# mycophonic/saprobe-alac

Hardware: AMD Instinct MI355X
Metric: Msamples/s decoded (16-bit stereo, 4096-frame packets) (higher is better)
Workload: dtype int32; 1 GPU; 65536 packets/GPU x 16-bit 2-ch 4096-frame ALAC, music-like synthetic, device-resident in/out; packets_per_gpu=65536

## Files before the change

saprobe-alac_amd/csrc/alac_duo.h:

```cpp
#ifndef ALAC_DUO_H
#define ALAC_DUO_H

#include <type_traits>

#include "alac_regular.h"

namespace alac {

#ifndef ALAC_WRAP_COUNTDOWN
#define ALAC_WRAP_COUNTDOWN 0
#endif
#ifndef ALAC_DUO_CHUNK
#define ALAC_DUO_CHUNK 16
#endif
constexpr uint32_t DUO_CHUNK = ALAC_DUO_CHUNK;
static_assert(DUO_CHUNK % 16u == 0u && DUO_CHUNK <= 32u, "a writer's half chunk is whole groups of 8 steps and fits a stager row");
constexpr int DUO_UN8_MAX = 12;
enum { ROLE_A = 0, ROLE_B = 1, ROLE_BOTH = 2, ROLE_C = 3 };

template <class W, class B, int NA, int OUT, int ROLE, bool F16, bool NARROW, bool EA, bool UN8W = false, bool EC = false, int WMODE = 0>
ALAC_DEV void duo_phase(W& wv, const DevCfg& cfg, const B& bits, RegLane<W>& s, uint32_t size, uint32_t ns,
                        uint32_t n_it, uint32_t hdr_pos, uint32_t den_shift, uint32_t chan_bits, int32_t mix_res,
                        uint32_t mix_sh, uint32_t na_rt, uint32_t shift_pos, uint32_t sb, uint32_t mode) {
    constexpr bool DO_A = ROLE == ROLE_A || ROLE == ROLE_BOTH, DO_B = ROLE == ROLE_B || ROLE == ROLE_BOTH;
    constexpr bool RAW = OUT == OUT_RAW;
    constexpr bool LAST = OUT == OUT_STEREO || OUT == OUT_MONO || RAW;
    constexpr bool CPE = OUT == OUT_STEREO;
    constexpr bool QND = W::kResMem || EC;
    constexpr bool GEN = NA == 0;
    constexpr int NR = GEN ? 1 : NA;
    constexpr bool WRAP = !(NA == 4 || NA == 5 || NA == 6 || NA == 8);
    constexpr uint32_t BIAS = 0x80000000u;
    static_assert(!(EA && EC), "one writer");
    constexpr bool DO_C = (ROLE == ROLE_C || ROLE == ROLE_BOTH) && EC;
    constexpr bool EMIT_A = (EA || EC) && LAST && !RAW;
    constexpr bool DO_EMIT = EMIT_A ? (EC ? DO_C : DO_A) : DO_B;
    constexpr uint32_t CH = EMIT_A ? DUO_CHUNK / 2u : DUO_CHUNK;
    constexpr bool U16_OUT = F16 && EC && OUT == OUT_UTILE;
    constexpr bool C16 = F16 && EC && CPE && EMIT_A;
    const uint32_t na = GEN ? na_rt : (uint32_t)NA;
#ifdef ALAC_SYNC_DIAG
    wv.dg_phase = LAST ? 1u : 0u;
#endif
    uint32_t kb = cfg.kb;
    ALAC_OWN_REG(kb);
    const uint32_t wb = go_shl(1u, kb) - 1u;
    const uint32_t c31kb = 31u - kb;
    const uint32_t chan_shift = 32u - chan_bits;
    const int32_t den_half = den_shift ? (int32_t)(1u << (den_shift - 1u)) : 0;
    const uint32_t rnd_neg = (1u << den_shift) - 1u;

    int32_t coef[NR];
    uint32_t hb[NR + 1];
    if (DO_B) {
#pragma unroll
        for (int j = 0; j < NR; ++j)
            coef[j] = (!GEN || ((uint32_t)j < na && na != 31)) ? (int32_t)(int16_t)bits.get(hdr_pos + 16u + 16u * (uint32_t)j, 16) : 0;
#pragma unroll
        for (int j = 0; j <= NR; ++j) hb[j] = BIAS;
    }
    uint64_t pk_acc = 0;
    uint32_t pk_n = 0;
    const uint32_t bps = cfg.bps;
    const uint64_t pk_msk = bps == 4 ? 0xffffffffull : ((1ull << (8u * bps)) - 1ull);
    const bool merge_any = DO_EMIT && LAST && !F16 && !RAW && wv.any(sb != 0);
    const bool mode_any = DO_B && wv.any(mode != 0);
    int32_t dprev = 0;
    auto prepass = [&](uint32_t idx, int32_t del) -> int32_t {
        if (!mode_any) return del;
        const int32_t dd = idx == 0 ? del : sext_cs(del + dprev, chan_shift);
        dprev = mode != 0 ? dd : dprev;
        return mode != 0 ? dd : del;
    };
    constexpr bool MID_ONLY = !NARROW && WMODE == 1;
    const bool mid = !NARROW && (MID_ONLY || !wv.any(ns != 0u && chan_bits > 25u));
    auto predict = [&](int32_t del, auto wrap) -> int32_t {
        constexpr bool WR = decltype(wrap)::value;
        if (NARROW) return predict_narrow<NR, GEN, WR, !RAW>(coef, hb, na, del, den_shift, den_half, rnd_neg, chan_shift);
        if (MID_ONLY || mid) return predict_narrow<NR, GEN, WR, !RAW, true>(coef, hb, na, del, den_shift, den_half, rnd_neg, chan_shift);
        if constexpr (!MID_ONLY) return predict_wide<NR, GEN, WR>(coef, hb, na, del, den_shift, den_half, chan_shift);
        return 0;
    };
    auto predict_q = [&](int32_t x, auto wrap) -> int32_t {
        constexpr bool WR = decltype(wrap)::value;
        if (!QND) return predict(x, wrap);
        if (NARROW) return predict_narrow_nd<NR, GEN, WR, !RAW>(coef, hb, na, (uint32_t)x, den_shift, den_half, rnd_neg, chan_shift);
        return predict(gol_unfold((uint32_t)x), wrap);
    };
    using wrap_yes = std::integral_constant<bool, WRAP>;
    using wrap_no = std::integral_constant<bool, false>;
    const uint32_t nzm = mix_res != 0 ? 0xffffffffu : 0u;

    uint32_t ns_live = s.err == 0 ? ns : 0u;
    if (DO_A) gol_head(s, c31kb);
    auto qval = [&](uint32_t nd) -> int32_t { return QND ? (int32_t)nd : gol_unfold(nd); };
    auto golomb_chunk = [&](uint32_t c) {
        const uint32_t buf = c & 1u;
        if ((c + 1u) * CH <= n_it) {
#pragma nounroll
            for (uint32_t g = 0; g < CH; g += GOL_TICK) {
                s.rd.tick(wv, s.pos);
                s.near = gol_near(s, c * CH + g, ns_live);
#pragma nounroll
                for (uint32_t h = g; h < g + GOL_TICK; h += 4u) {
#pragma unroll
                    for (uint32_t j = 0; j < 4u; ++j)
                        wv.rq_write(buf, h + j, qval(gol_step<true>(wv, bits, s, size, kb, wb, c31kb, chan_bits, c * CH + h + j, ns, ns_live)));
                }
            }
            return;
        }
#pragma nounroll
        for (uint32_t j = 0; j < CH; ++j) {
            const uint32_t i = c * CH + j;
            if (i >= n_it) break;
            if ((i & (GOL_TICK - 1u)) == 0) {
                s.rd.tick(wv, s.pos);
                s.near = gol_near(s, i, ns_live);
            }
            wv.rq_write(buf, j, qval(gol_step<true>(wv, bits, s, size, kb, wb, c31kb, chan_bits, i, ns, ns_live)));
        }
    };
    constexpr bool FP_OK = F16 && CPE && LAST && !EMIT_A && !RAW;
    uint32_t fp_base = 0, fp_inc = 0;
    using fp_yes = std::integral_constant<bool, true>;
    using fp_no = std::integral_constant<bool, false>;
    auto emit = [&](uint32_t i, int32_t o, int32_t u, uint64_t sw, uint32_t jj, auto fp) {
        constexpr bool FP = decltype(fp)::value;
        const bool on = i < ns;
        if (RAW) {
            wv.st_push_if((uint32_t)o, on);
            return;
        }
        int32_t l = o, r = 0;
        if (CPE) {
            const int32_t vv = o;
            const int32_t mv = NARROW ? ALAC_MUL24(mix_res, vv) : (int32_t)((uint32_t)mix_res * (uint32_t)vv);
            l = u + (int32_t)((uint32_t)vv & nzm) - (mv >> mix_sh);
            r = (int32_t)((((uint32_t)(l - vv)) & nzm) | ((uint32_t)vv & ~nzm));
        }
        if (F16) {
            const uint32_t pcm = ((uint32_t)l & 0xffffu) | ((uint32_t)r << 16);
            if (FP) wv.st_put(fp_base, jj, pcm, fp_inc);
            else wv.st_push_if(pcm, on);
            return;
        }
        if (cfg.bit_depth == 20) {
            l = (int32_t)((uint32_t)l << 4);
            r = (int32_t)((uint32_t)r << 4);
        }
        if (merge_any) {
            const uint32_t sh_l = sb ? (uint32_t)(sw >> (64u - sb)) : 0u;
            const uint32_t sh_r = (CPE && sb) ? (uint32_t)((sw << sb) >> (64u - sb)) : 0u;
            l = (int32_t)((uint32_t)l << sb) | (int32_t)sh_l;
            r = (int32_t)((uint32_t)r << sb) | (int32_t)sh_r;
        }
        {
            pk_acc |= ((uint64_t)(uint32_t)l & pk_msk) << (8u * pk_n);
            pk_n += on ? bps : 0u;
            bool em = pk_n >= 4u;
            wv.st_push_if((uint32_t)pk_acc, em);
            pk_acc = em ? pk_acc >> 32 : pk_acc;
            pk_n = em ? pk_n - 4u : pk_n;
            if (CPE) {
                pk_acc |= ((uint64_t)(uint32_t)r & pk_msk) << (8u * pk_n);
                pk_n += on ? bps : 0u;
                em = pk_n >= 4u;
                wv.st_push_if((uint32_t)pk_acc, em);
                pk_acc = em ? pk_acc >> 32 : pk_acc;
                pk_n = em ? pk_n - 4u : pk_n;
            }
            pk_acc &= pk_n ? ((1ull << (8u * pk_n)) - 1ull) : 0ull;
        }
    };
    uint32_t u_even = 0;
    auto put = [&](uint32_t buf, uint32_t j, uint32_t i, int32_t o, int32_t u, uint64_t sw, uint32_t jj, auto fp) {
#pragma unroll
        for (int t = NR; t >= 1; --t) hb[t] = hb[t - 1];
        hb[0] = (uint32_t)o ^ BIAS;
        if (!LAST && U16_OUT) {
            if (i & 1u) *wv.u_row(i >> 1) = (int32_t)ALAC_PACK_LO16(u_even, o);
            else if (i + 1u == n_it) *wv.u_row(i >> 1) = o;
            else u_even = (uint32_t)o;
        } else if (!LAST) *wv.u_row(i) = o;
        else if (EMIT_A) wv.rq_write(buf, CH + j, o);
        else emit(i, o, u, sw, jj, fp);
    };
    constexpr bool PK3 = CPE && LAST && !F16 && !RAW && !EMIT_A;
    constexpr bool PK3C = CPE && LAST && !F16 && !RAW && EMIT_A && EC;
    const bool sb8 = (PK3 || PK3C) && !wv.any(ns != 0u && sb != 8u);
    const bool sb0 = (PK3 || PK3C) && !wv.any(ns != 0u && sb != 0u);
    const bool pk3 = (PK3 || PK3C) && bps == 3u && (sb8 || sb0);
    const uint32_t sh_byte = shift_pos >> 3, sh_bit = shift_pos & 7u;
    auto pk3_block = [&](uint32_t rowq, const int32_t (&vv4)[4], const int32_t (&uu4)[4], uint32_t g0, uint32_t g1, uint32_t g2) {
        const uint32_t w0 = (uint32_t)(((((uint64_t)g0) << 32) | g1) << sh_bit >> 32);
        const uint32_t w1 = (uint32_t)(((((uint64_t)g1) << 32) | g2) << sh_bit >> 32);
        uint32_t lq[4], rq[4];
#pragma unroll
        for (uint32_t j = 0; j < 4u; ++j) {
            const int32_t vv = vv4[j];
            const int32_t mv = NARROW ? ALAC_MUL24(mix_res, vv) : (int32_t)((uint32_t)mix_res * (uint32_t)vv);
            int32_t l = uu4[j] + (int32_t)((uint32_t)vv & nzm) - (mv >> mix_sh);
            int32_t r = (int32_t)((((uint32_t)(l - vv)) & nzm) | ((uint32_t)vv & ~nzm));
            if (sb8) {
                const uint32_t w = j < 2u ? w0 : w1;
// ... 235 lines not shown
                        for (uint32_t j = 0; j < UN; ++j) {
                            const int32_t o = predict_q(dv[j], wrap);
#pragma unroll
                            for (int t = NR; t >= 1; --t) hb[t] = hb[t - 1];
                            hb[0] = (uint32_t)o ^ BIAS;
                            if (j & 1u) ub[(ptrdiff_t)(j >> 1) * rs] = (int32_t)ALAC_PACK_LO16(u_even, o);
                            else u_even = (uint32_t)o;
                        }
                        continue;
                    }
#pragma unroll
                    for (uint32_t j = 0; j < UN; ++j)
                        put(buf, g + j, c * CH + g + j, predict_q(dv[j], wrap), uv[j], sv[j], j, fp);
                    if (FP) wv.st_advance(fp_inc);
                    if (LAST && !EMIT_A) wv.st_step();
                }
            };
            auto run_groups = [&](auto wrap) {
                if (FP_OK) {
                    const uint32_t c_end = (c + 1u) * CH;
                    const bool ends_here = ns > c * CH && ns < c_end;
                    if (!wv.any(ends_here)) {
                        fp_inc = ns >= c_end ? UN : 0u;
                        groups(wrap, fp_yes{});
                        return;
                    }
                    groups(wrap, fp_no{});
                    if (ends_here) (void)wv.st_finish();
                    return;
                }
                groups(wrap, fp_no{});
            };
#if !ALAC_WRAP_COUNTDOWN
            if (WRAP) {
                constexpr uint32_t T = 32767u - CH;
                uint32_t far = 0;
#pragma unroll
                for (int j = 0; j < NR; ++j) far = umax(far, (uint32_t)coef[j] + T);
                if (!wv.any(far > 2u * T)) {
                    run_groups(wrap_no{});
                    return;
                }
            }
#else
            if (WRAP) {
                if (wrap_safe == 0u) {
                    uint32_t mag = 0;
#pragma unroll
                    for (int j = 0; j < NR; ++j) mag = umax(mag, (uint32_t)(coef[j] ^ (coef[j] >> 31)));
                    wrap_safe = (32767u - wv.max_u32(mag)) / CH;
                }
                if (wrap_safe != 0u) {
                    --wrap_safe;
                    run_groups(wrap_no{});
                    return;
                }
            }
#endif
            run_groups(wrap_yes{});
            return;
        }
#if ALAC_WRAP_COUNTDOWN
        wrap_safe = 0;
#endif
#pragma nounroll
        for (uint32_t j = 0; j < CH; ++j) {
            const uint32_t i = c * CH + j;
            if (i >= n_it) break;
            const int32_t qv = wv.rq_read(buf, j);
            const int32_t del = prepass(i, QND ? gol_unfold((uint32_t)qv) : qv);
            int32_t o;
            if (i == 0 || (GEN && na == 0)) o = del;
            else if (i <= na || (GEN && na == 31)) o = sext_cs(del + (int32_t)(hb[0] ^ BIAS), chan_shift);
            else o = predict(del, wrap_yes{});
            put(buf, j, i, o, (CPE && !EMIT_A) ? *wv.u_row(i) : 0,
                (!EMIT_A && merge_any) ? bits.window_raw(shift_pos + i * sstep) : 0ull, 0u, fp_no{});
            if (LAST && !EMIT_A) wv.st_step();
            if (FP_OK && i + 1u == ns) (void)wv.st_finish();
        }
    };

    const uint32_t nch = (n_it + CH - 1u) / CH;
    const uint32_t iters = nch + (EMIT_A ? 2u : 1u);
    for (uint32_t c = 0; c < iters; ++c) {
        if (DO_A) {
            if (EMIT_A && !EC && c >= 2u) fetch_chunk(c - 2u);
            if (c < nch) golomb_chunk(c);
        }
        if (DO_B) {
            if (c >= 1u && c <= nch) predict_chunk(c - 1u);
        }
        if (DO_A && EMIT_A && !EC) {
            if (c >= 2u) emit_chunk(c - 2u);
        }
        if (DO_C && C16) {
            if (c >= 2u) emit_chunk16(c - 2u);
            if (c >= 1u && c <= nch) fetch_u16(c - 1u);
        } else if (DO_C && EMIT_A) {
            if (c >= 2u) {
#pragma unroll
                for (uint32_t j = 0; j < CH; ++j) {
                    u_v[j] = u_n[j];
                    sw_v[j] = sw_n[j];
                }
#pragma unroll
                for (uint32_t q = 0; q < CH / 4u; ++q) {
                    g_v[q][0] = g_n[q][0];
                    g_v[q][1] = g_n[q][1];
                    g_v[q][2] = g_n[q][2];
                }
            }
            if (c >= 1u && c <= nch) fetch_mem_ahead(c - 1u);
            if (c >= 2u) {
                fetch_chunk(c - 2u);
                emit_chunk(c - 2u);
            }
        }
        wv.duo_sync();
    }
    if (DO_EMIT && LAST) wv.st_tail(pk_acc, pk_n);
    if (!LAST) wv.duo_sync_mem();
}

template <class W, class B, int T, int OUT, int LPP, int NAC = 0, bool U16 = false>
ALAC_DEV void duo_phase_lanes(W& wv, const B& bits, uint32_t q, uint32_t n_it, uint32_t hdr_pos, uint32_t den_shift,
                              uint32_t chan_bits, uint32_t na_rt) {
    static_assert(LPP == 2 || LPP == 4, "lanes per packet");
    static_assert(LPP == 2 ? NAC == 0 : (NAC >= 1 && (NAC + 3) / 4 == T), "four lanes: T = ceil(order / 4)");
    const uint32_t na = NAC != 0 ? (uint32_t)NAC : na_rt;
    constexpr bool LAST = OUT != OUT_UTILE;
    constexpr uint32_t CH = LAST ? DUO_CHUNK / 2u : DUO_CHUNK;
    constexpr uint32_t BIAS = 0x80000000u;
    const bool wraps = order_wraps16(na);
    const uint32_t chan_shift = 32u - chan_bits;
    const int32_t den_half = den_shift ? (int32_t)(1u << (den_shift - 1u)) : 0;
    const int32_t dh0 = q == 0u ? den_half : 0;
    const uint32_t rnd_neg = (1u << den_shift) - 1u;
    const uint32_t q0m = q == 0u ? 0xffffffffu : 0u;
    const uint32_t up1 = q < 3u ? 0xffffffffu : 0u, up2 = q < 2u ? 0xffffffffu : 0u, up3 = q < 1u ? 0xffffffffu : 0u;
    int32_t coef[T], wneg[T], m[T];
    uint32_t g[T + 1];
#pragma unroll
    for (int t = 0; t < T; ++t) {
        const uint32_t jt = q * (uint32_t)T + (uint32_t)t;
        const bool have = jt < na;
        coef[t] = have ? (int32_t)(int16_t)bits.get(hdr_pos + 16u + 16u * jt, 16) : 0;
        wneg[t] = have ? -(int32_t)(na - jt) : 0;
        m[t] = have ? 1 : 0;
        g[t] = BIAS;
    }
    g[T] = BIAS;
    int32_t prev = 0;
    constexpr int QTOP = NAC != 0 ? (NAC - 1) / T : 1, TTOP = NAC != 0 ? NAC - QTOP * T : T;
    const bool top_last = na == 2u * (uint32_t)T;

    auto step = [&](uint32_t i, uint32_t nd, auto plain_c, auto wrap_c) -> int32_t {
        constexpr bool PLAIN = decltype(plain_c)::value, WR = decltype(wrap_c)::value;
        uint32_t topb;
        if constexpr (LPP == 2) topb = wv.pair_hi(top_last ? g[T] : g[T - 1]);
        else topb = wv.template quad_from<QTOP>(g[TTOP]);
        const uint32_t nsg = nd & 1u, sgnm = 0u - nsg, hm = nd >> 1;
        const int32_t del = (int32_t)(hm ^ sgnm);
        int32_t rem = (int32_t)(hm + nsg);
        if (!PLAIN) {
            if (i <= na) rem = 0;
        }
        const uint32_t rnd = rnd_neg & sgnm;
        int32_t acc = dh0, s = 0;
        int32_t e[T], sg[T];
        uint32_t qv[T];
#pragma unroll
        for (int t = T - 1; t >= 0; --t) {
            e[t] = (int32_t)(g[t] - topb);
            const uint32_t ae = ALAC_SAD(topb, g[t], rnd);
            sg[t] = ALAC_SIGN(e[t]);
            qv[t] = ae >> den_shift;
            if (t != 0) {
                acc = ALAC_MAD24(coef[t], e[t], acc);
                s = ALAC_MAD24(qv[t], wneg[t], s);
            } else {
                acc = ALAC_MUL24(coef[t], e[t]) + acc;
                s = ALAC_MUL24((int32_t)qv[t], wneg[t]) + s;
            }
        }
        if (LPP == 2) rem += (int32_t)(wv.pair_hi((uint32_t)s) & q0m);
        else rem += (int32_t)((wv.template quad_up<1>((uint32_t)s) & up1) + (wv.template quad_up<2>((uint32_t)s) & up2) +
                              (wv.template quad_up<3>((uint32_t)s) & up3));
#pragma unroll
        for (int t = T - 1; t >= 0; --t) {
            const int32_t go = ALAC_MED3_0(rem, m[t]);
            const int32_t delta = (int32_t)ALAC_XAD(sg[t], sgnm, nsg);
            rem = ALAC_MAD24(qv[t], wneg[t], rem);
            int32_t cj = ALAC_MAD24(delta, go, coef[t]);
            if (WR) cj = (int32_t)(int16_t)cj;
            coef[t] = cj;
        }
        const int32_t at = LPP == 2 ? wv.pair_sum(acc) : wv.quad_sum(acc);
        int32_t o = ALAC_SEXT_BITS(del + (int32_t)(topb ^ BIAS) + (at >> den_shift), chan_bits);
        if (!PLAIN) {
            if (i == 0u) o = del;
            else if (i <= na) o = sext_cs(del + prev, chan_shift);
        }
// ... 280 lines not shown
```

saprobe-alac_amd/csrc/alac_regular.h:

```cpp
#ifndef ALAC_REGULAR_H
#define ALAC_REGULAR_H

#include "alac_wave.h"

#ifndef ALAC_NOINLINE
#define ALAC_NOINLINE
#endif
#ifndef ALAC_UNLIKELY
#define ALAC_UNLIKELY(x) __builtin_expect(!!(x), 0)
#endif
#ifndef ALAC_HD
#define ALAC_HD ALAC_DEV
#endif
#ifndef ALAC_SAD
#define ALAC_SAD(a, b, c) (((a) > (b) ? (a) - (b) : (b) - (a)) + (c))
#endif
#ifndef ALAC_LOAD4
#define ALAC_LOAD4(q, a, b, c, d) \
    do {                         \
        (a) = (q)[0];            \
        (b) = (q)[1];            \
        (c) = (q)[2];            \
        (d) = (q)[3];            \
    } while (0)
// ... 48 lines not shown
#endif
#ifndef ALAC_NOT_ADD
#define ALAC_NOT_ADD(a, c) (~(uint32_t)(a) + (uint32_t)(c))
#endif
#ifndef ALAC_ALIGNBIT
#define ALAC_ALIGNBIT(hi, lo, sh) ((uint32_t)(((((uint64_t)(uint32_t)(hi)) << 32) | (uint32_t)(lo)) >> ((sh) & 31u)))
#endif
#ifndef ALAC_MULHI
#define ALAC_MULHI(a, b) ((uint32_t)(((uint64_t)(uint32_t)(a) * (uint64_t)(uint32_t)(b)) >> 32))
#endif
#ifndef ALAC_BFE
#define ALAC_BFE(x, off, width) ((((uint32_t)(x)) >> ((off) & 31u)) & ((1u << ((width) & 31u)) - 1u))
#endif
#ifndef ALAC_PACK_LO16
#define ALAC_PACK_LO16(x, y) ((((uint32_t)(x)) & 0xffffu) | (((uint32_t)(y)) << 16))
#endif
#ifndef ALAC_PACK_HI16
#define ALAC_PACK_HI16(x, y) ((((uint32_t)(x)) >> 16) | (((uint32_t)(y)) & 0xffff0000u))
#endif
#ifndef ALAC_PK_ADD16
#define ALAC_PK_ADD16(a, b) \
    (((((uint32_t)(a)) + ((uint32_t)(b))) & 0xffffu) | (((((uint32_t)(a)) >> 16) + (((uint32_t)(b)) >> 16)) << 16))
#endif
#ifndef ALAC_PK_SUB16
#define ALAC_PK_SUB16(a, b) \
    (((((uint32_t)(a)) - ((uint32_t)(b))) & 0xffffu) | (((((uint32_t)(a)) >> 16) - (((uint32_t)(b)) >> 16)) << 16))
#endif

namespace alac {

constexpr uint32_t KEY_WIDE = 1024;
constexpr uint32_t KEY_IRREGULAR = 2048;
constexpr uint32_t NUM_KEYS = 2049;

ALAC_DEV bool regular_order(uint32_t na) { return na <= 16 || na == 31; }
ALAC_DEV int32_t imax(int32_t a, int32_t b) { return a > b ? a : b; }

ALAC_HD bool lean_config(const DevCfg& cfg) { return cfg.kb != 0 && cfg.pb <= 73u; }

ALAC_DEV uint32_t classify_regular(const DevCfg& cfg, const uint8_t* pkt, uint32_t size, uint32_t avail) {
    if (cfg.num_channels > 2 || cfg.aligned16 == 0 || !lean_config(cfg) ||
        cfg.frame_length > 65536u || cfg.frame_length <= 32u)
        return KEY_IRREGULAR;
    const Bits bits{pkt, size, avail};
    if (size < 12) return KEY_IRREGULAR;
    const uint32_t tag = bits.get(0, 3);
    const bool cpe = cfg.num_channels == 2;
    if (cpe ? tag != 1 : !(tag == 0 || tag == 3)) return KEY_IRREGULAR;
    if (bits.get(7, 12) != 0) return KEY_IRREGULAR;
    const uint32_t hdr = bits.get(19, 4);
    if (hdr & 1u) return KEY_IRREGULAR;
    const uint32_t bs = (hdr >> 1) & 3u;
    if (bs == 3) return KEY_IRREGULAR;
    const uint32_t chan_bits = cfg.bit_depth - 8u * bs + (cpe ? 1u : 0u);
    if (chan_bits < 1 || chan_bits > 33 || cfg.bit_depth < 8u * bs) return KEY_IRREGULAR;
    const uint32_t wide = chan_bits > 23u ? KEY_WIDE : 0u;
    uint32_t pos = 23;
    uint32_t ns = cfg.frame_length;
    if (hdr >> 3) {
        ns = bits.get(pos, 32);
        pos += 32;
    }
    if (ns == 0 || ns > cfg.frame_length) return KEY_IRREGULAR;
    pos += 16;
    const uint32_t hu = bits.get(pos, 16);
    const uint32_t nu = hu & 0x1fu;
    if ((hu >> 12) != 0 || !regular_order(nu)) return KEY_IRREGULAR;
    pos += 16u + 16u * nu;
    uint32_t nv = 0;
    if (cpe) {
        const uint32_t hv = bits.get(pos, 16);
        nv = hv & 0x1fu;
        if ((hv >> 12) != 0 || !regular_order(nv)) return KEY_IRREGULAR;
        pos += 16u + 16u * nv;
    }
    const uint64_t ent = (uint64_t)pos + (uint64_t)bs * 8u * (cpe ? 2u : 1u) * ns;
    if ((ent >> 3) >= size || (bs != 0 && (ent >> 3) + 10u > size)) return KEY_IRREGULAR;
    return nu * 32u + nv + wide;
}

#ifndef ALAC_RING_START_AHEAD
#define ALAC_RING_START_AHEAD 0
#endif
template <class W>
struct RingRd {
    const uint32_t* base;
    uint32_t bias;
    uint32_t end_b;
    uint32_t full;
    uint32_t wa, wb;
    uint32_t fill;
    static constexpr uint32_t RING = W::kRingDw;
    static_assert(RING >= 32, "blocks of 8 dwords need a ring of 32");
    uint32_t p0, p1, p2, p3, p4, p5, p6, p7;
    bool pend;

    ALAC_DEV void init(const uint8_t* pkt, uint32_t size) {
        const uint32_t mis = (uint32_t)(reinterpret_cast<uintptr_t>(pkt) & 3u);
        base = reinterpret_cast<const uint32_t*>(pkt - mis);
        bias = mis * 8u;
        end_b = size ? mis + size : 0u;
        full = end_b >> 2;
        wa = wb = fill = 0;
        p0 = p1 = p2 = p3 = p4 = p5 = p6 = p7 = 0;
        pend = false;
    }
    ALAC_DEV uint32_t tail1(uint32_t idx) const {
        const uint32_t last = end_b ? (end_b - 1u) >> 2 : 0u;
        const uint32_t v = base[umin(idx, last)];
        const uint32_t lo = idx * 4u;
        const uint32_t nb = end_b > lo ? umin(end_b - lo, 4u) : 0u;
        return v & (nb >= 4u ? 0xffffffffu : ((1u << (8u * nb)) - 1u));
    }
    ALAC_DEV void load8(uint32_t at) {
        if (at + 8u <= full) {
            ALAC_LOAD4(base + at, p0, p1, p2, p3);
            ALAC_LOAD4(base + at + 4u, p4, p5, p6, p7);
        } else {
            p0 = tail1(at);
            p1 = tail1(at + 1u);
            p2 = tail1(at + 2u);
            p3 = tail1(at + 3u);
            p4 = tail1(at + 4u);
            p5 = tail1(at + 5u);
            p6 = tail1(at + 6u);
            p7 = tail1(at + 7u);
        }
    }
    ALAC_DEV void commit(W& wv) {
        const uint32_t slot = fill & (RING - 1u);
        const uint32_t d0 = __builtin_bswap32(p0);
        wv.ring_write4(slot, d0, __builtin_bswap32(p1), __builtin_bswap32(p2), __builtin_bswap32(p3));
        wv.ring_write4((fill + 4u) & (RING - 1u), __builtin_bswap32(p4), __builtin_bswap32(p5), __builtin_bswap32(p6),
                       __builtin_bswap32(p7));
        wv.ring_write1(slot == 0u ? RING : RING + 1u, d0);
        fill += 8u;
        pend = false;
    }
    ALAC_DEV void start(W& wv, uint32_t posb) {
        const uint32_t ni = posb >> 5;
        fill = ni & ~7u;
        pend = false;
#if ALAC_RING_START_AHEAD
        uint32_t blk[3][8];
#pragma unroll
        for (uint32_t b = 0; b < 3u; ++b) {
            load8(fill + 8u * b);
            blk[b][0] = p0, blk[b][1] = p1, blk[b][2] = p2, blk[b][3] = p3;
            blk[b][4] = p4, blk[b][5] = p5, blk[b][6] = p6, blk[b][7] = p7;
        }
#pragma unroll
        for (uint32_t b = 0; b < 3u; ++b) {
            p0 = blk[b][0], p1 = blk[b][1], p2 = blk[b][2], p3 = blk[b][3];
            p4 = blk[b][4], p5 = blk[b][5], p6 = blk[b][6], p7 = blk[b][7];
            commit(wv);
        }
#else
#pragma nounroll
        for (int b = 0; b < 3; ++b) {
            load8(fill);
            commit(wv);
        }
#endif
        reseek(wv, posb);
    }
    ALAC_DEV void reseek(W& wv, uint32_t posb) {
        const uint32_t ni = posb >> 5;
        while (fill < ni + 12u) {
            if (!pend) load8(fill);
            commit(wv);
        }
        wv.ring_read2(ni & (RING - 1u), wa, wb);
    }
    ALAC_DEV uint64_t window64(W& wv, uint32_t posb) {
        const uint32_t ni = posb >> 5, r = posb & 31u;
        while (fill < ni + 4u) {
            if (!pend) load8(fill);
            commit(wv);
        }
        const uint64_t a = wv.ring_read(ni & (RING - 1u)), b = wv.ring_read((ni + 1u) & (RING - 1u));
        const uint64_t c = wv.ring_read((ni + 2u) & (RING - 1u));
        const uint64_t hi = (a << 32) | b;
        return r ? (hi << r) | (c >> (32u - r)) : hi;
    }
    ALAC_DEV void tick(W& wv, uint32_t posb) {
        if (pend) commit(wv);
        if (fill + 8u <= (posb >> 5) + RING) {
            load8(fill);
            pend = true;
        }
    }
};

constexpr uint32_t GOL_PARK = 0x40000000u;

template <class W>
struct RegLane {
    RingRd<W> rd;
    uint32_t pos;
    uint32_t mean, zmode, pb, max_pos;
    uint32_t zq;
    uint32_t pbs;
    uint32_t h_sh, h_ck, h_t9, h_norun;
    uint32_t near;
    int32_t err;
    ALAC_DEV uint32_t upos() const { return pos + 1u - rd.bias; }
    ALAC_DEV void set_upos(uint32_t p) { pos = p + rd.bias - 1u; }
    ALAC_DEV void set_pb(uint32_t p) {
        pb = p;
        pbs = p << 23;
    }
};

constexpr uint32_t GOL_TICK = 8;
constexpr uint32_t GOL_REACH = 41u * GOL_TICK;
template <class W>
ALAC_DEV uint32_t gol_near(const RegLane<W>& s, uint32_t i, uint32_t ns_live) {
    return ALAC_SUBSAT(s.pos + (GOL_REACH + 1u), s.max_pos) | ALAC_SUBSAT(i + GOL_TICK + 1u, ns_live) | s.zmode;
}

template <class W, class B>
ALAC_DEV uint32_t golomb_slow(W& wv, const B& bits, RegLane<W>& s, uint32_t size, uint32_t kb, uint32_t wb,
                              uint32_t chan_bits, uint32_t i, uint32_t ns, uint32_t& ns_live) {
    if (i >= ns_live) {
        s.zq = GOL_PARK - 1u;
        return 0u;
    }
    const uint32_t bias = s.rd.bias;
    uint32_t pos = s.upos(), mean = s.mean, zmode = s.zmode, zrem = s.zq + 1u;
    const uint32_t max_pos = s.max_pos - bias;
    int32_t err = 0;
    uint32_t ndq = 0;
    if (pos >= max_pos) {
        err = ST_OVERRUN;
    } else {
        uint32_t m = mean >> 9;
        const uint32_t k = umin(31u - clz32(m + 3u), kb);
        m = (1u << k) - 1u;
        const uint32_t w = (uint32_t)(s.rd.window64(wv, pos + bias) >> 32);
        uint32_t n = clz32(~w);
        if (n >= 9) {
            const uint32_t gpos = pos + 9u;
            const uint32_t gb = gpos & 7u;
            const bool five = chan_bits + gb > 32u;
            if ((gpos >> 3) > size || (five && (gpos >> 3) >= size)) err = ST_MALFORMED;
            const uint64_t w2 = s.rd.window64(wv, gpos + bias);
            if (chan_bits == 0) n = 0;
            else if (chan_bits <= 32) n = (uint32_t)(w2 >> (64u - chan_bits));
            else n = (uint32_t)(w2 >> 31) & ((2u << gb) - 1u);
            pos += 9u + chan_bits;
        } else {
            const uint32_t v = (w << (n + 1u)) >> (32u - k);
            pos += n + 1u + k - (v >= 2 ? 0u : 1u);
            n = v >= 2 ? n * m + v - 1u : n * m;
        }
        if (err == 0) {
            const uint32_t nd = n + zmode;
            ndq = nd == 0xffffffffu ? 0u : nd;
            mean = s.pb * nd + mean - ((s.pb * mean) >> 9);
            if (n > 0xffffu) mean = 0xffffu;
            zmode = 0;
            if ((mean << 2) < 512u && i + 1u < ns) {
                zmode = 1;
                int32_t k32 = (int32_t)clz32(mean) - 24 + (int32_t)((mean + 16u) >> 6);
                if (k32 < 0) k32 = 0;
                const uint32_t kz = (uint32_t)k32;
                const uint32_t mz = ((1u << kz) - 1u) & wb;
                if ((pos >> 3) > size) {
                    err = ST_MALFORMED;
                } else {
                    const uint32_t wz = (uint32_t)(s.rd.window64(wv, pos + bias) >> 32);
                    const uint32_t pre = clz32(~wz);
                    uint32_t rl;
                    if (pre >= 9) {
                        rl = (wz << 9) >> 16;
                        pos += 25u;
                    } else {
                        const uint32_t val = kz == 0 ? 0u : (wz << (pre + 1u)) >> (32u - kz);
                        pos += pre + kz + (val < 2 ? 0u : 1u);
                        rl = val < 2 ? pre * mz : pre * mz + val - 1u;
                    }
                    if ((uint64_t)i + 1u + rl > ns) err = ST_SAMPLE_OVERRUN;
                    zrem = rl;
                    if (rl >= 65535u) zmode = 0;
                    mean = 0;
                }
            }
        }
    }
    if (err == 0) {
        s.set_upos(pos);
        s.mean = mean;
        s.zmode = zmode;
        s.zq = zrem - 1u;
        s.near = ALAC_SUBSAT(pos + bias + GOL_REACH, s.max_pos) | ALAC_SUBSAT(i + GOL_TICK + 1u, ns_live) | zmode;
        return ndq;
    }
    s.err = err;
    s.zq = GOL_PARK - 1u;
    ns_live = 0u;
    return 0u;
}

template <class W>
ALAC_DEV void gol_head(RegLane<W>& s, uint32_t c31kb) {
    s.h_sh = ~s.pos;
    s.h_norun = (uint32_t)((int32_t)s.zq >> 31);
    s.h_t9 = ALAC_MULHI(s.mean, s.pbs);
    s.h_ck = (uint32_t)imax((int32_t)ALAC_FFBH((s.mean >> 9) + 3u), (int32_t)c31kb);
}

template <bool ESC, class W, class B>
ALAC_DEV uint32_t gol_step(W& wv, const B& bits, RegLane<W>& s, uint32_t size, uint32_t kb, uint32_t wb, uint32_t c31kb,
                           uint32_t chan_bits, uint32_t i, uint32_t ns, uint32_t& ns_live) {
    const uint32_t o_pos = s.pos, o_mean = s.mean, o_zq = s.zq;
    RingRd<W>& rd = s.rd;
    const uint32_t o_wa = rd.wa, o_wb = rd.wb;
    uint32_t n, esc, mt, pos2, aoff, zq2, mean2, nhi;
    uint32_t rare, sh2, ck2, t92, norun2;
    {
        const uint32_t ck = s.h_ck, norun = s.h_norun;
        const uint32_t w = ALAC_ALIGNBIT(o_wa, o_wb, s.h_sh);
        const uint32_t k = 31u - ck;
        const uint32_t nw = ~w;
        mt = o_mean - s.h_t9;
        const uint32_t pre = ALAC_FFBH(nw);
        zq2 = ALAC_NOT_ADD(norun, o_zq);
        const uint32_t off = ck - pre;
        esc = ALAC_SUBSAT(pre, 8u);
        const uint32_t v = ALAC_BFE(w, off, k);
        uint32_t pk = pre << k;
        const uint32_t c2 = v > 1u ? 1u : 0u;
        const uint32_t vm1 = ALAC_SUBSAT(v, 1u);
        pk -= pre;
        const uint32_t cons = pre + k + c2;
        n = pk + vm1;
        const uint32_t cm = cons & norun;
        n &= norun;
        pos2 = o_pos + cm;
        mean2 = ALAC_MULU24(s.pb, n) + mt;
        aoff = pos2 >> 3;
        nhi = n >> 16;
        aoff &= 4u * (RingRd<W>::RING - 1u);
    }
    wv.ring_read2_at(aoff, rd.wa, rd.wb);
    {
        const uint32_t zs = ALAC_SUBSAT(128u, mean2);
        uint32_t x = mean2 >> 9;
        sh2 = ~pos2;
        const uint32_t fl = esc | nhi | zs;
        t92 = ALAC_MULHI(mean2, s.pbs);
        x += 3u;
        norun2 = (uint32_t)((int32_t)zq2 >> 31);
        x = ALAC_FFBH(x);
        rare = (fl | s.near) & s.h_norun;
        ck2 = (uint32_t)imax((int32_t)x, (int32_t)c31kb);
    }
    s.pos = pos2;
    s.mean = mean2;
    s.zq = zq2;
    s.h_sh = sh2;
    s.h_ck = ck2;
    s.h_t9 = t92;
    s.h_norun = norun2;
    uint32_t ndq = n;
    if (ALAC_UNLIKELY(wv.any(rare != 0u))) {
        if (rare != 0u) {
            bool done = false;
            if (ESC && s.near == 0u) {
                if (esc != 0u && chan_bits <= 32u && chan_bits != 0u) {
                    const uint64_t hi = (((uint64_t)o_wa) << 32) | o_wb;
                    const uint32_t o_wc = wv.ring_read(((o_pos >> 5) + 2u) & (RingRd<W>::RING - 1u));
                    const uint32_t r1 = (o_pos & 31u) + 1u;
                    const uint64_t w64 = r1 < 32u ? (hi << r1) | ((uint64_t)o_wc >> (32u - r1))
                                                  : ((((uint64_t)o_wb) << 32) | o_wc);
                    const uint32_t n2 = (uint32_t)((w64 << 9) >> (64u - chan_bits));
                    const uint32_t m2 = n2 > 0xffffu ? 0xffffu : s.pb * n2 + mt;
                    if (m2 >= 128u) {
                        s.pos = o_pos + 9u + chan_bits;
                        s.mean = m2;
                        ndq = n2 == 0xffffffffu ? 0u : n2;
                        done = true;
                    }
                } else if (esc == 0u && (n >> 16) != 0u) {
                    s.mean = 0xffffu;
                    done = true;
                }
            }
            if (!done) {
                s.pos = o_pos;
                s.mean = o_mean;
                s.zq = o_zq;
                ndq = golomb_slow(wv, bits, s, size, kb, wb, chan_bits, i, ns, ns_live);
            }
            rd.reseek(wv, s.pos);
            gol_head(s, c31kb);
        }
    }
    return ndq;
}

ALAC_DEV int32_t gol_unfold(uint32_t nd) { return (int32_t)((nd >> 1) ^ (0u - (nd & 1u))); }

#ifndef ALAC_TAP_ORDER
#define ALAC_TAP_ORDER 2
#endif
template <int NR, bool GEN, bool WRAP, bool CB_POS = false, bool MID = false>
ALAC_DEV int32_t predict_narrow_core(int32_t (&coef)[NR], const uint32_t (&hb)[NR + 1], uint32_t na, int32_t del, uint32_t sgnm,
                                     uint32_t nsg, int32_t rem, uint32_t den_shift, int32_t den_half, uint32_t rnd_neg,
                                     uint32_t chan_shift) {
    constexpr uint32_t BIAS = 0x80000000u;
    uint32_t topb = hb[NR];
    if (GEN) {
#pragma unroll
        for (int j = 1; j < NR; ++j)
            if (na == (uint32_t)j) ALAC_PICK(topb, hb[j]);
    }
    const uint32_t rnd = rnd_neg & sgnm;
    int32_t accx = 0;
    uint32_t ntx = 0u - (topb ^ sgnm);
    ALAC_OWN_REG(ntx);
    int32_t gos = 1;
#pragma unroll
    for (int j = NR - 1; j >= 0; --j) {
        if (GEN && (uint32_t)j >= na) continue;
#if ALAC_TAP_ORDER == 1
        const int32_t ex = (int32_t)ALAC_XAD(hb[j], sgnm, ntx);
        const uint32_t ae = ALAC_SAD(topb, hb[j], rnd);
        const int32_t delta = ALAC_SIGN(ex);
        accx = MID ? (int32_t)((uint32_t)accx + (uint32_t)coef[j] * (uint32_t)ex)
                   : ALAC_MAD24(coef[j], ex, accx);
        const uint32_t q = ae >> den_shift;
        int32_t go = ALAC_CLAMP01(rem);
        if (MID) {
            go &= gos;
            gos = go;
        }
        rem = MID ? (int32_t)((uint32_t)rem - q * (na - (uint32_t)j)) : ALAC_MSUB24(rem, q, na - (uint32_t)j);
        const int32_t cj = ALAC_MAD24(delta, go, coef[j]);
        coef[j] = WRAP ? (int32_t)(int16_t)cj : cj;
#else
        const uint32_t ae = ALAC_SAD(topb, hb[j], rnd);
        const int32_t ex = (int32_t)((hb[j] ^ sgnm) + ntx);
        int32_t go = ALAC_CLAMP01(rem);
        if (MID) {
            go &= gos;
            gos = go;
        }
        const int32_t delta = ALAC_SIGN(ex);
        const uint32_t q = ae >> den_shift;
        accx = MID ? (int32_t)((uint32_t)accx + (uint32_t)coef[j] * (uint32_t)ex)
                   : ALAC_MAD24(coef[j], ex, accx);
        rem = MID ? (int32_t)((uint32_t)rem - q * (na - (uint32_t)j)) : ALAC_MSUB24(rem, q, na - (uint32_t)j);
        const int32_t cj = ALAC_MAD24(delta, go, coef[j]);
        coef[j] = WRAP ? (int32_t)(int16_t)cj : cj;
#endif
    }
#if ALAC_TAP_ORDER == 1
    const int32_t acc = (int32_t)ALAC_XAD(accx, sgnm, nsg + (uint32_t)den_half);
#else
    const int32_t acc = (int32_t)(((uint32_t)accx ^ sgnm) + (nsg + (uint32_t)den_half));
#endif
    const int32_t o = del + (int32_t)(topb ^ BIAS) + (acc >> den_shift);
    return CB_POS ? ALAC_SEXT_BITS(o, 32u - chan_shift) : sext_cs(o, chan_shift);
}

template <int NR, bool GEN, bool WRAP, bool CB_POS = false, bool MID = false>
ALAC_DEV int32_t predict_narrow(int32_t (&coef)[NR], const uint32_t (&hb)[NR + 1], uint32_t na, int32_t del,
                                uint32_t den_shift, int32_t den_half, uint32_t rnd_neg, uint32_t chan_shift) {
    const uint32_t sgnm = (uint32_t)(del >> 31), nsg = (uint32_t)del >> 31;
    return predict_narrow_core<NR, GEN, WRAP, CB_POS, MID>(coef, hb, na, del, sgnm, nsg, (int32_t)(((uint32_t)del ^ sgnm) + nsg), den_shift,
                                                      den_half, rnd_neg, chan_shift);
}
template <int NR, bool GEN, bool WRAP, bool CB_POS = false>
ALAC_DEV int32_t predict_narrow_nd(int32_t (&coef)[NR], const uint32_t (&hb)[NR + 1], uint32_t na, uint32_t nd,
                                   uint32_t den_shift, int32_t den_half, uint32_t rnd_neg, uint32_t chan_shift) {
// ... 109 lines not shown
```

saprobe-alac_amd/csrc/k_dec16l.hip:

```cpp
#define ALAC_LDS_ROWS 32
#define ALAC_LDS_FLUSH 32
#define ALAC_WRAP_COUNTDOWN 1
#define ALAC_DUO_CHUNK 32
#define ALAC_RING_START_AHEAD 1
#include "alac_gpu.h"

#define ALAC_DECODE_KERNEL alac_decode_16l
#define ALAC_DECODE_WIDE 0
#define ALAC_DECODE_DEPTH 16
#define ALAC_DECODE_GATED 0
#define ALAC_DECODE_ROLES 4
#define ALAC_DECODE_WAVES 4
#define ALAC_DECODE_NO_LANES 1

namespace alack {

#include "k_decode_body.inc"

}
```

Before: 276,200 Msamples/s.

## Split Golomb decode into far and end forms to drop per-step bounds checks

Adds an ALAC_LEAN_ENDS switch, enabled for the 16-bit lanes kernel. It runs the main Golomb loop in a 'far' form while the bit position is provably distant from the packet end, so the per-tick byte-distance test drops out of the near flag, and uses an 'end' form with an explicit per-step bound test only for the remaining chunks. It also simplifies the sample-end near test and splits ring-buffer tail block loads into separate fetch and mask passes. The cost is more code paths and template instantiations, with a risk of correctness problems at packet boundaries if the reach bounds are wrong.

```diff
diff --git a/saprobe-alac_amd/csrc/alac_duo.h b/saprobe-alac_amd/csrc/alac_duo.h
--- a/saprobe-alac_amd/csrc/alac_duo.h
+++ b/saprobe-alac_amd/csrc/alac_duo.h
@@ -94,6 +94,38 @@
     uint32_t ns_live = s.err == 0 ? ns : 0u;
     if (DO_A) gol_head(s, c31kb);
     auto qval = [&](uint32_t nd) -> int32_t { return QND ? (int32_t)nd : gol_unfold(nd); };
+#if ALAC_LEAN_PACKET_END
+    auto golomb_chunk = [&](uint32_t c, auto form) {
+        constexpr int FORM = decltype(form)::value;
+        const uint32_t buf = c & 1u;
+        if (FORM == GOL_FORM_FAR || (c + 1u) * CH <= n_it) {
+#pragma nounroll
+            for (uint32_t g = 0; g < CH; g += GOL_TICK) {
+                s.rd.tick(wv, s.pos);
+                s.near = gol_near_rest(s, c * CH + g, ns_live);
+#pragma nounroll
+                for (uint32_t h = g; h < g + GOL_TICK; h += 4u) {
+#pragma unroll
+                    for (uint32_t j = 0; j < 4u; ++j)
+                        wv.rq_write(buf, h + j, qval(gol_step<true, FORM>(wv, bits, s, size, kb, wb, c31kb, chan_bits, c * CH + h + j, ns, ns_live)));
+                }
+            }
+            return;
+        }
+        if constexpr (FORM != GOL_FORM_FAR) {
+#pragma nounroll
+            for (uint32_t j = 0; j < CH; ++j) {
+                const uint32_t i = c * CH + j;
+                if (i >= n_it) break;
+                if ((i & (GOL_TICK - 1u)) == 0) {
+                    s.rd.tick(wv, s.pos);
+                    s.near = gol_near_rest(s, i, ns_live);
+                }
+                wv.rq_write(buf, j, qval(gol_step<true, FORM>(wv, bits, s, size, kb, wb, c31kb, chan_bits, i, ns, ns_live)));
+            }
+        }
+    };
+#else
     auto golomb_chunk = [&](uint32_t c) {
         const uint32_t buf = c & 1u;
         if ((c + 1u) * CH <= n_it) {
@@ -121,6 +153,7 @@
             wv.rq_write(buf, j, qval(gol_step<true>(wv, bits, s, size, kb, wb, c31kb, chan_bits, i, ns, ns_live)));
         }
     };
+#endif
     constexpr bool FP_OK = F16 && CPE && LAST && !EMIT_A && !RAW;
     uint32_t fp_base = 0, fp_inc = 0;
     using fp_yes = std::integral_constant<bool, true>;
@@ -522,10 +555,11 @@
 
     const uint32_t nch = (n_it + CH - 1u) / CH;
     const uint32_t iters = nch + (EMIT_A ? 2u : 1u);
-    for (uint32_t c = 0; c < iters; ++c) {
+#if ALAC_LEAN_PACKET_END
+    auto iteration = [&](uint32_t c, auto form) {
         if (DO_A) {
             if (EMIT_A && !EC && c >= 2u) fetch_chunk(c - 2u);
-            if (c < nch) golomb_chunk(c);
+            if (c < nch) golomb_chunk(c, form);
         }
         if (DO_B) {
             if (c >= 1u && c <= nch) predict_chunk(c - 1u);
@@ -557,7 +591,53 @@
             }
         }
         wv.duo_sync();
-    }
+    };
+    uint32_t c_far = 0;
+    if (DO_A) {
+        for (; (c_far + 1u) * CH <= n_it; ++c_far) {
+            if (wv.any(c_far * CH < ns_live && !gol_far(s, CH))) break;
+            iteration(c_far, std::integral_constant<int, GOL_FORM_FAR>{});
+        }
+    }
+    for (uint32_t c = c_far; c < iters; ++c) iteration(c, std::integral_constant<int, GOL_FORM_END>{});
+#else
+    for (uint32_t c = 0; c < iters; ++c) {
+        if (DO_A) {
+            if (EMIT_A && !EC && c >= 2u) fetch_chunk(c - 2u);
+            if (c < nch) golomb_chunk(c);
+        }
+        if (DO_B) {
+            if (c >= 1u && c <= nch) predict_chunk(c - 1u);
+        }
+        if (DO_A && EMIT_A && !EC) {
+            if (c >= 2u) emit_chunk(c - 2u);
+        }
+        if (DO_C && C16) {
+            if (c >= 2u) emit_chunk16(c - 2u);
+            if (c >= 1u && c <= nch) fetch_u16(c - 1u);
+        } else if (DO_C && EMIT_A) {
+            if (c >= 2u) {
+#pragma unroll
+                for (uint32_t j = 0; j < CH; ++j) {
+                    u_v[j] = u_n[j];
+                    sw_v[j] = sw_n[j];
+                }
+#pragma unroll
+                for (uint32_t q = 0; q < CH / 4u; ++q) {
+                    g_v[q][0] = g_n[q][0];
+                    g_v[q][1] = g_n[q][1];
+                    g_v[q][2] = g_n[q][2];
+                }
+            }
+            if (c >= 1u && c <= nch) fetch_mem_ahead(c - 1u);
+            if (c >= 2u) {
+                fetch_chunk(c - 2u);
+                emit_chunk(c - 2u);
+            }
+        }
+        wv.duo_sync();
+    }
+#endif
     if (DO_EMIT && LAST) wv.st_tail(pk_acc, pk_n);
     if (!LAST) wv.duo_sync_mem();
 }
diff --git a/saprobe-alac_amd/csrc/alac_regular.h b/saprobe-alac_amd/csrc/alac_regular.h
--- a/saprobe-alac_amd/csrc/alac_regular.h
+++ b/saprobe-alac_amd/csrc/alac_regular.h
@@ -154,6 +154,12 @@
 #ifndef ALAC_RING_START_AHEAD
 #define ALAC_RING_START_AHEAD 0
 #endif
+#ifndef ALAC_LEAN_ENDS
+#define ALAC_LEAN_ENDS 0
+#endif
+#define ALAC_LEAN_PACKET_END ((ALAC_LEAN_ENDS & 1) != 0)
+#define ALAC_LEAN_SAMPLE_END ((ALAC_LEAN_ENDS & 2) != 0)
+#define ALAC_LEAN_TAIL_BLOCKS ((ALAC_LEAN_ENDS & 4) != 0)
 template <class W>
 struct RingRd {
     const uint32_t* base;
@@ -184,10 +190,68 @@
         const uint32_t nb = end_b > lo ? umin(end_b - lo, 4u) : 0u;
         return v & (nb >= 4u ? 0xffffffffu : ((1u << (8u * nb)) - 1u));
     }
+#if ALAC_LEAN_TAIL_BLOCKS
+    ALAC_DEV uint32_t tail_fetch(uint32_t idx) const {
+        const uint32_t last = end_b ? (end_b - 1u) >> 2 : 0u;
+        return base[umin(idx, last)];
+    }
+    ALAC_DEV uint32_t tail_mask(uint32_t idx) const {
+        const uint32_t lo = idx * 4u;
+        const uint32_t nb = end_b > lo ? umin(end_b - lo, 4u) : 0u;
+        return nb >= 4u ? 0xffffffffu : ((1u << (8u * nb)) - 1u);
+    }
+    ALAC_DEV void fetch8(uint32_t at) {
+        if (at + 8u <= full) {
+            ALAC_LOAD4(base + at, p0, p1, p2, p3);
+            ALAC_LOAD4(base + at + 4u, p4, p5, p6, p7);
+        } else {
+            p0 = tail_fetch(at);
+            p1 = tail_fetch(at + 1u);
+            p2 = tail_fetch(at + 2u);
+            p3 = tail_fetch(at + 3u);
+            p4 = tail_fetch(at + 4u);
+            p5 = tail_fetch(at + 5u);
+            p6 = tail_fetch(at + 6u);
+            p7 = tail_fetch(at + 7u);
+        }
+    }
+    ALAC_DEV void mask8(uint32_t at) {
+        if (at + 8u > full) {
+            p0 &= tail_mask(at);
+            p1 &= tail_mask(at + 1u);
+            p2 &= tail_mask(at + 2u);
+            p3 &= tail_mask(at + 3u);
+            p4 &= tail_mask(at + 4u);
+            p5 &= tail_mask(at + 5u);
+            p6 &= tail_mask(at + 6u);
+            p7 &= tail_mask(at + 7u);
+        }
+    }
+#endif
     ALAC_DEV void load8(uint32_t at) {
         if (at + 8u <= full) {
             ALAC_LOAD4(base + at, p0, p1, p2, p3);
             ALAC_LOAD4(base + at + 4u, p4, p5, p6, p7);
+#if ALAC_LEAN_TAIL_BLOCKS
+        } else {
+            p0 = tail_fetch(at);
+            p1 = tail_fetch(at + 1u);
+            p2 = tail_fetch(at + 2u);
+            p3 = tail_fetch(at + 3u);
+            p4 = tail_fetch(at + 4u);
+            p5 = tail_fetch(at + 5u);
+            p6 = tail_fetch(at + 6u);
+            p7 = tail_fetch(at + 7u);
+            p0 &= tail_mask(at);
+            p1 &= tail_mask(at + 1u);
+            p2 &= tail_mask(at + 2u);
+            p3 &= tail_mask(at + 3u);
+            p4 &= tail_mask(at + 4u);
+            p5 &= tail_mask(at + 5u);
+            p6 &= tail_mask(at + 6u);
+            p7 &= tail_mask(at + 7u);
+        }
+#else
         } else {
             p0 = tail1(at);
             p1 = tail1(at + 1u);
@@ -198,6 +262,7 @@
             p6 = tail1(at + 6u);
             p7 = tail1(at + 7u);
         }
+#endif
     }
     ALAC_DEV void commit(W& wv) {
         const uint32_t slot = fill & (RING - 1u);
@@ -217,7 +282,11 @@
         uint32_t blk[3][8];
 #pragma unroll
         for (uint32_t b = 0; b < 3u; ++b) {
+#if ALAC_LEAN_TAIL_BLOCKS
+            fetch8(fill + 8u * b);
+#else
             load8(fill + 8u * b);
+#endif
             blk[b][0] = p0, blk[b][1] = p1, blk[b][2] = p2, blk[b][3] = p3;
             blk[b][4] = p4, blk[b][5] = p5, blk[b][6] = p6, blk[b][7] = p7;
         }
@@ -225,6 +294,9 @@
         for (uint32_t b = 0; b < 3u; ++b) {
             p0 = blk[b][0], p1 = blk[b][1], p2 = blk[b][2], p3 = blk[b][3];
             p4 = blk[b][4], p5 = blk[b][5], p6 = blk[b][6], p7 = blk[b][7];
+#if ALAC_LEAN_TAIL_BLOCKS
+            mask8(fill);
+#endif
             commit(wv);
         }
 #else
@@ -286,12 +358,28 @@
 
 constexpr uint32_t GOL_TICK = 8;
 constexpr uint32_t GOL_REACH = 41u * GOL_TICK;
+ALAC_DEV uint32_t gol_near_samples(uint32_t i, uint32_t ns_live) {
+#if ALAC_LEAN_SAMPLE_END
+    return ALAC_SUBSAT((i | (GOL_TICK - 1u)) + 1u, ns_live);
+#else
+    return ALAC_SUBSAT(i + GOL_TICK + 1u, ns_live);
+#endif
+}
 template <class W>
 ALAC_DEV uint32_t gol_near(const RegLane<W>& s, uint32_t i, uint32_t ns_live) {
-    return ALAC_SUBSAT(s.pos + (GOL_REACH + 1u), s.max_pos) | ALAC_SUBSAT(i + GOL_TICK + 1u, ns_live) | s.zmode;
-}
-
-template <class W, class B>
+    return ALAC_SUBSAT(s.pos + (GOL_REACH + 1u), s.max_pos) | gol_near_samples(i, ns_live) | s.zmode;
+}
+enum { GOL_FORM_NEAR = 0, GOL_FORM_FAR = 1, GOL_FORM_END = 2 };
+#if ALAC_LEAN_PACKET_END
+constexpr uint32_t GOL_ESC_REACH = 64;
+constexpr uint32_t GOL_STEP_MAX = 72;
+template <class W>
+ALAC_DEV bool gol_far(const RegLane<W>& s, uint32_t steps) { return ALAC_SUBSAT(s.pos + (GOL_STEP_MAX * steps + 1u), s.max_pos) == 0u; }
+#endif
+template <class W>
+ALAC_DEV uint32_t gol_near_rest(const RegLane<W>& s, uint32_t i, uint32_t ns_live) { return gol_near_samples(i, ns_live) | s.zmode; }
+
+template <class W, class B, int FORM = GOL_FORM_NEAR>
 ALAC_DEV uint32_t golomb_slow(W& wv, const B& bits, RegLane<W>& s, uint32_t size, uint32_t kb, uint32_t wb,
                               uint32_t chan_bits, uint32_t i, uint32_t ns, uint32_t& ns_live) {
     if (i >= ns_live) {
@@ -337,7 +425,11 @@
                 int32_t k32 = (int32_t)clz32(mean) - 24 + (int32_t)((mean + 16u) >> 6);
                 if (k32 < 0) k32 = 0;
                 const uint32_t kz = (uint32_t)k32;
+#if ALAC_LEAN_PACKET_END
+                const uint32_t mz = (1u << umin(kz, kb)) - 1u;
+#else
                 const uint32_t mz = ((1u << kz) - 1u) & wb;
+#endif
                 if ((pos >> 3) > size) {
                     err = ST_MALFORMED;
                 } else {
@@ -365,7 +457,7 @@
         s.mean = mean;
         s.zmode = zmode;
         s.zq = zrem - 1u;
-        s.near = ALAC_SUBSAT(pos + bias + GOL_REACH, s.max_pos) | ALAC_SUBSAT(i + GOL_TICK + 1u, ns_live) | zmode;
+        s.near = (FORM != GOL_FORM_NEAR ? 0u : ALAC_SUBSAT(pos + bias + GOL_REACH, s.max_pos)) | gol_near_samples(i, ns_live) | zmode;
         return ndq;
     }
     s.err = err;
@@ -382,9 +474,10 @@
     s.h_ck = (uint32_t)imax((int32_t)ALAC_FFBH((s.mean >> 9) + 3u), (int32_t)c31kb);
 }
 
-template <bool ESC, class W, class B>
+template <bool ESC, int FORM = GOL_FORM_NEAR, class W, class B>
 ALAC_DEV uint32_t gol_step(W& wv, const B& bits, RegLane<W>& s, uint32_t size, uint32_t kb, uint32_t wb, uint32_t c31kb,
                            uint32_t chan_bits, uint32_t i, uint32_t ns, uint32_t& ns_live) {
+    static_assert(FORM == GOL_FORM_NEAR || ALAC_LEAN_PACKET_END, "the other forms come with the switch");
     const uint32_t o_pos = s.pos, o_mean = s.mean, o_zq = s.zq;
     RingRd<W>& rd = s.rd;
     const uint32_t o_wa = rd.wa, o_wb = rd.wb;
@@ -420,7 +513,10 @@
         const uint32_t zs = ALAC_SUBSAT(128u, mean2);
         uint32_t x = mean2 >> 9;
         sh2 = ~pos2;
-        const uint32_t fl = esc | nhi | zs;
+        uint32_t fl = esc | nhi | zs;
+#if ALAC_LEAN_PACKET_END
+        if (FORM == GOL_FORM_END) fl |= ALAC_SUBSAT(o_pos + 2u, s.max_pos);
+#endif
         t92 = ALAC_MULHI(mean2, s.pbs);
         x += 3u;
         norun2 = (uint32_t)((int32_t)zq2 >> 31);
@@ -439,7 +535,12 @@
     if (ALAC_UNLIKELY(wv.any(rare != 0u))) {
         if (rare != 0u) {
             bool done = false;
-            if (ESC && s.near == 0u) {
+#if ALAC_LEAN_PACKET_END
+            const bool inside = s.near == 0u && (FORM != GOL_FORM_END || ALAC_SUBSAT(o_pos + (GOL_ESC_REACH + 1u), s.max_pos) == 0u);
+#else
+            const bool inside = s.near == 0u;
+#endif
+            if (ESC && inside) {
                 if (esc != 0u && chan_bits <= 32u && chan_bits != 0u) {
                     const uint64_t hi = (((uint64_t)o_wa) << 32) | o_wb;
                     const uint32_t o_wc = wv.ring_read(((o_pos >> 5) + 2u) & (RingRd<W>::RING - 1u));
@@ -463,7 +564,7 @@
                 s.pos = o_pos;
                 s.mean = o_mean;
                 s.zq = o_zq;
-                ndq = golomb_slow(wv, bits, s, size, kb, wb, chan_bits, i, ns, ns_live);
+                ndq = golomb_slow<W, B, FORM>(wv, bits, s, size, kb, wb, chan_bits, i, ns, ns_live);
             }
             rd.reseek(wv, s.pos);
             gol_head(s, c31kb);
diff --git a/saprobe-alac_amd/csrc/k_dec16l.hip b/saprobe-alac_amd/csrc/k_dec16l.hip
--- a/saprobe-alac_amd/csrc/k_dec16l.hip
+++ b/saprobe-alac_amd/csrc/k_dec16l.hip
@@ -3,6 +3,9 @@
 #define ALAC_WRAP_COUNTDOWN 1
 #define ALAC_DUO_CHUNK 32
 #define ALAC_RING_START_AHEAD 1
+#ifndef ALAC_LEAN_ENDS
+#define ALAC_LEAN_ENDS 7
+#endif
 #include "alac_gpu.h"
 
 #define ALAC_DECODE_KERNEL alac_decode_16l
```

New measurement: 282,500 Msamples/s, median of 6. +2.3%, better.
